# SerezD/vqvae-vqgan-pytorch-lightning

Hardware: AMD Instinct MI355X
Metric: images/sec/node (256x256 bs=32/GPU) VQ-VAE train step (higher is better)
Workload: dtype bf16; 1 GPU; standard_vqvae cb=1024, 256x256 bs=32/GPU (encoder+VQ+decoder fwd/bwd + AdamW); yaml=example_confs/standard_vqvae.yaml, global_batch=32, parallelism=dp1, launch=hipGraph replay (fwd+bwd) + eager all-reduce + AdamW, deterministic=False

## Files before the change

include/vqk.h:

```cpp
#ifndef VQK_H_
#define VQK_H_

#include <stddef.h>
#include <stdint.h>

#ifdef __cplusplus
extern "C" {
#endif

#define VQK_F32 0
#define VQK_BF16 1

enum vqk_status {
    VQK_OK = 0,
    VQK_ERR_SHAPE = -1,
    VQK_ERR_DTYPE = -2,
    VQK_ERR_ALIGN = -3,
    VQK_ERR_LAUNCH = -4,
    VQK_ERR_ARG = -5,
    VQK_ERR_WORKSPACE = -6
};

const char* vqk_status_str(int status);
int vqk_version(void);
// ... 162 lines not shown
int vqk_ctx_set_tile_queue(vqk_ctx* ctx, void* ws, int64_t ws_bytes);
int vqk_ctx_set_deterministic(vqk_ctx* ctx, int on, void* ws, int64_t ws_bytes);
int vqk_set_tuning(const char* name, int value);
int vqk_reset_tuning(void);
int vqk_tuning_count(void);
const char* vqk_tuning_name(int i);
int vqk_conv_set_block_caps(int stream_blocks, int wgrad_blocks);
int vqk_probe_stream_add(const float* src, float* dst, int64_t bytes, int blocks, int passes, int sleep, void* stream);
int vqk_calib_fill(void* w, int64_t bytes, void* stream);
int vqk_calib_mfma(const void* w, int64_t w_bytes, float* sink, int iters, int blocks, void* stream);
int64_t vqk_calib_mfma_flops(int iters, int blocks);
int vqk_calib_copy(const void* src, void* dst, int64_t bytes, void* stream);
int vqk_conv_pack_dgrad(const float* w, void* wt, int dtype, int cout, int cin, int ksize, void* stream);
int vqk_conv2d_wgrad(int dtype, const void* x, const void* dy, float* dw, int n, int h_in, int w_in, int cin,
                     int cout, int ksize, int ups, const void* zeros, void* stream);
int64_t vqk_conv2d_wgrad_edge_ws_bytes(void);
int vqk_conv2d_wgrad_edge(int dtype, const void* x, const void* dy, float* dw, void* ws, int64_t ws_bytes, int n, int h,
                          int w, int cin, int cout, const void* zeros, void* stream);
int vqk_conv2d_wgrad_edge_true(int dtype, const void* x, const void* dy, float* dw, void* ws, int64_t ws_bytes, int n, int h,
                               int w, int cin, int cout, int thin_true, const void* zeros, void* stream);
int vqk_conv2d_thin_out(int dtype, const void* x, const void* w, const float* bias, void* y, int n, int h, int wd, int cin,
                        int cout, int act, const void* zeros, void* stream);
int vqk_colsum(int dtype, const void* x, int64_t rows, int c, float* out, void* stream);
int vqk_colsum_lead(int dtype, const void* x, int64_t rows, int c, int c_out, float scale, float* out, void* stream);
int vqk_cast(const float* src, void* dst, int dtype, int64_t n, void* stream);

int vqk_gn_stats(int dtype, const void* x, int n, int64_t hw, int c, int groups, float eps,
                 double* acc, float* stats, void* stream);
int vqk_gn_apply(int dtype, const void* x, const float* stats, const float* w, const float* b, void* y,
                 int n, int64_t hw, int c, int groups, int silu, void* stream);
// ... 135 lines not shown
```

vqvae-vqgan-pytorch-lightning_amd/_native.py:

```python
from __future__ import annotations

import ctypes
import fcntl
import os
import subprocess
from ctypes import c_char_p, c_double, c_float, c_int, c_int32, c_int64, c_void_p, POINTER

_HERE = os.path.dirname(os.path.abspath(__file__))
_CSRC = os.path.join(_HERE, 'csrc')
_SO = os.environ.get('VQK_LIB') or os.path.join(_HERE, 'libvqk.so')
_lib = None

P = c_void_p
I, L, F = c_int, c_int64, c_float

_PROTOS = {
    'vqk_row_sqnorm_f32': [P, L, I, P, P],
    'vqk_vq_assign_f32': [P, P, P, P, L, I, I, I, P, P],
    'vqk_vq_assign_filtered_f32': [P, P, P, P, L, I, I, I, P, P, L, P],
    'vqk_probe_stream_add': [P, P, L, I, I, I, P],
    'vqk_calib_fill': [P, L, P],
    'vqk_calib_mfma': [P, L, P, I, I, P],
    'vqk_calib_copy': [P, P, L, P],
    'vqk_vq_prepare_f32': [P, I, I, P, L, P],
# ... 53 lines not shown
    'vqk_conv_set_variant': [I],
    'vqk_conv_set_block_caps': [I, I],
    'vqk_set_deterministic': [I, P, L],
    'vqk_set_scratch': [P, L],
    'vqk_set_tile_queue': [P, L],
    'vqk_ctx_create': [P],
    'vqk_ctx_destroy': [P],
    'vqk_ctx_make_current': [P],
    'vqk_ctx_set_scratch': [P, P, L],
    'vqk_ctx_set_tile_queue': [P, P, L],
    'vqk_ctx_set_deterministic': [P, I, P, L],
    'vqk_conv_pack_dgrad': [P, P, I, I, I, I, P],
    'vqk_conv2d_wgrad': [I, P, P, P, I, I, I, I, I, I, I, P, P],
    'vqk_conv2d_wgrad_pooled_dy': [I, P, P, P, I, I, I, I, I, F, P, P],
    'vqk_conv2d_wgrad_ups_phase': [I, P, P, P, I, I, I, I, I, F, P, P],
    'vqk_split_pair_f32': [P, P, L, I, P],
    'vqk_conv2d_fprop_x3_gnstats': [P, P, P, P, P, I, I, I, I, I, I, P, I, P, P],
    'vqk_conv2d_wgrad_x3': [P, P, P, I, I, I, I, I, I, F, P, P],
    'vqk_conv2d_wgrad_x3_f32': [P, P, P, I, I, I, I, I, I, F, P],
    'vqk_conv2d_wgrad_pooled_dy_phase': [I, P, P, P, I, I, I, I, I, F, P, P],
    'vqk_conv2d_wgrad_edge': [I, P, P, P, P, L, I, I, I, I, I, P, P],
    'vqk_conv2d_wgrad_edge_true': [I, P, P, P, P, L, I, I, I, I, I, I, P, P],
    'vqk_conv2d_thin_out': [I, P, P, P, P, I, I, I, I, I, I, P, P],
    'vqk_colsum': [I, P, L, I, P, P],
    'vqk_colsum_lead': [I, P, L, I, I, F, P, P],
    'vqk_cast': [P, P, I, L, P],
    'vqk_gn_stats': [I, P, I, L, I, I, F, P, P, P],
    'vqk_gn_apply': [I, P, P, P, P, P, I, L, I, I, I, P],
    'vqk_gn_forward': [I, P, P, P, P, P, P, I, L, I, I, F, I, P],
    'vqk_gn_forward_presummed': [I, P, P, P, P, P, P, I, L, I, I, F, I, P],
# ... 131 lines not shown
```

vqvae-vqgan-pytorch-lightning_amd/csrc/api.cpp:

```cpp
#include <stdint.h>
#include <new>
#include "common.h"

extern "C" {

const char* vqk_status_str(int status) {
    switch (status) {
        case VQK_OK: return "ok";
        case VQK_ERR_SHAPE: return "unsupported or inconsistent shape";
        case VQK_ERR_DTYPE: return "unsupported dtype";
        case VQK_ERR_ALIGN: return "pointer is not 16-byte aligned";
        case VQK_ERR_LAUNCH: return "kernel launch failed";
        case VQK_ERR_ARG: return "bad argument";
        case VQK_ERR_WORKSPACE: return "workspace too small";
        default: return "unknown status";
    }
}

int vqk_version(void) { return 1; }
const char* vqk_arch(void) { return "gfx950"; }

}

struct vqk_ctx {
// ... 83 lines not shown
    {"SK_MAXMB", 0, 0},
    {"UPS_PHASE", 0, 0},
    {"WGRAD_BLOCKS", 0, 0},
    {"WGMX", 0, 0},
    {"WGRAD_GEN_BLOCKS", 0, 0},
    {"WGRAD_NO_PW16", 0, 0},
    {"WGRAD_NO_P16K", 0, 0},
    {"MX_HALF", 0, 0},
    {"MX_HALF_HW", 0, 0},
    {"UPFIRDN_TILE", 0, 0},
    {"GN_BLOCKS_REDUCE", 0, 0},
    {"GN_BLOCKS_APPLY", 0, 0},
    {"GN_NT_MB", 0, 0},
    {"GN_NO_SMALL", 0, 0},
    {"WGMX_COEF_E4", 0, 0},
    {"GN_CLUSTER_MAX_HW", 0, 0},
    {"COMM_CUS", 0, 0},
    {"MX_QUARTER", 0, 0},
    {"MX_S2", 0, 0},
    {"MX_S2_DGRAD_MIN", 0, 0},
    {"VQ_LDS", 0, 0},
    {"UPS_MERGE", 0, 0},
    {"TILE_QUEUE", 0, 0},
    {"X3_WL", 0, 0},
    {"X3_WGRAD_COEF_E4", 0, 0},
    {"X3_WGRAD_FOLD", 0, 0},
    {"X3_WGRAD_PHASE", 0, 0},
    {"X3_WGRAD_PHASE_CAP_PCT", 0, 0},
    {"X3_WGRAD_PHASE_COEF_E4", 0, 0}
};
// ... 28 lines not shown
```

vqvae-vqgan-pytorch-lightning_amd/csrc/conv_geom.h:

```cpp
#pragma once
#include "common.h"

namespace vqkd {

struct ConvGeom {
    int n, h_in, w_in, h, w, cin, cout, ks, ups;
    int stride, pad, zs, vh, vw;
    float acc_scale, out_gain;
    int pool;
    float pool_scale;
    int m;
    int sub, sub_py, sub_px, sub_h, sub_w, nkh, nkw, khl[2], kwl[2];
    int wrow_chunks;
    int cpt;
    int kchunks;
    int tiles_m, tiles_n;
    double* gn_ws;
    int gn_cpg;
    int gn_part_nblk, gn_part_base;
    int ntap, tap_oy, tap_ox, src_s, src_a, src_b, dst_s, dst_a, dst_b;
    int tapw, dst_h, dst_w, s2;
    int phase_mode;
    int phase_rev;
    int dy_pool;
// ... 22 lines not shown
int& conv_force_variant();
int& conv_wgrad_blocks();

int launch_conv3x3_x3(const void* x, const void* w, const float* bias, const void* res, void* y, const void* zeros,
                      const ConvGeom& g, int act, int blocks_cap, hipStream_t st);
int launch_conv3x3_wgrad_x3(const void* x, const void* dy, float* dw, const ConvGeom& g, int blocks_cap, hipStream_t st);

int launch_conv3x3_thin_out_f32(const float* x, const float* w, const float* bias, const float* res, float* y, int n, int h, int wd,
                                int cin, int act, float acc_scale, float out_gain, hipStream_t st);
int launch_conv3x3_thin_in_f32(const float* x, const float* w, const float* bias, float* y, int n, int h, int wd, int cout, hipStream_t st);
int thin_wgrad_rows(int h, int w);
int launch_conv3x3_wgrad_thin_f32(int mode, const float* wide, const float* thin, float* dw, int n, int h, int w, int cw, float scale,
                                  hipStream_t st);

int launch_conv3x3_wgrad_mx(const void* x, const void* dy, float* dw, const void* zeros, const ConvGeom& g, int tiles,
                            int splits, int pps, hipStream_t st, float* part = nullptr);

}
```

vqvae-vqgan-pytorch-lightning_amd/csrc/conv_wgmx.hip:

```cpp
#include "conv_geom.h"

namespace {
using vqkd::ConvGeom;
using vqkd::xcd_remap;

#ifndef VQK_WGMX_NST
#define VQK_WGMX_NST 3
#endif
#ifndef VQK_WGMX_PIN
#define VQK_WGMX_PIN 1
#endif
#define SGB(mask, n) __builtin_amdgcn_sched_group_barrier(mask, n, 0)

__device__ __forceinline__ void glds16(const void* src, char* lds_wave_base) {
    __builtin_amdgcn_global_load_lds((const VQK_GLB void*)src, (VQK_LDS void*)lds_wave_base, 16, 0, 0);
}
__device__ __forceinline__ bf16x8_t tr_frag2(const char* p) {
    const s16x4 lo = __builtin_amdgcn_ds_read_tr16_b64_v4i16((VQK_LDS s16x4*)p);
    const s16x4 hi = __builtin_amdgcn_ds_read_tr16_b64_v4i16((VQK_LDS s16x4*)(p + 256));
    typedef __attribute__((ext_vector_type(8))) short s16x8;
    const s16x8 v = {lo[0], lo[1], lo[2], lo[3], hi[0], hi[1], hi[2], hi[3]};
    return __builtin_bit_cast(bf16x8_t, v);
}

// ... 227 lines not shown
    }
}

__global__ __launch_bounds__(256) void wgrad_mx_reduce_kernel(const float* __restrict__ part, float* __restrict__ dw, int tiles,
                                                              int splits, int cin) {
    const int tile = blockIdx.y, tiles_ci = cin >> 6;
    const int e = (int)(blockIdx.x * 256 + threadIdx.x);
    if (e >= 64 * 9 * 64) return;
    const int cil = e & 63, ct = e >> 6, col = ct / 9, t = ct - col * 9;
    const int tco = tile / tiles_ci, tci = tile - tco * tiles_ci;
    float s = 0.0f;
    for (int k = 0; k < splits; ++k) s += part[((int64_t)k * tiles + tile) * (64 * 9 * 64) + e];
    dw[((int64_t)(tco * 64 + col) * 9 + t) * cin + tci * 64 + cil] += s;
}

}

namespace vqkd {

int launch_conv3x3_wgrad_mx(const void* x, const void* dy, float* dw, const void* zeros, const ConvGeom& g, int tiles,
                            int splits, int pps, hipStream_t st, float* part) {
    if (g.fold && (g.dy_pool || part)) return VQK_ERR_ARG;
    if (g.dy_pool >= 2) {
        if (g.dy_pool > 7 || part || (g.dy_pool >= 6 && (splits & 3))) return VQK_ERR_ARG;
        static const hipError_t attr4 = hipFuncSetAttribute((const void*)conv3x3_wgrad_mx_kernel<4>,
                                                            hipFuncAttributeMaxDynamicSharedMemorySize, VQK_WGMX_NST * 40960);
        if (attr4 != hipSuccess) return VQK_ERR_LAUNCH;
        hipLaunchKernelGGL(conv3x3_wgrad_mx_kernel<4>, dim3((unsigned)tiles, (unsigned)splits), dim3(512), VQK_WGMX_NST * 40960, st,
                           (const bf16_raw*)x, (const bf16_raw*)dy, dw, (const char*)zeros, g, pps, part);
        return hipGetLastError() == hipSuccess ? VQK_OK : VQK_ERR_LAUNCH;
    }
    static const hipError_t attr = hipFuncSetAttribute((const void*)conv3x3_wgrad_mx_kernel<9>,
                                                       hipFuncAttributeMaxDynamicSharedMemorySize, VQK_WGMX_NST * 40960);
    (void)attr;
    hipLaunchKernelGGL(conv3x3_wgrad_mx_kernel<9>, dim3((unsigned)tiles, (unsigned)splits), dim3(512), VQK_WGMX_NST * 40960, st,
                       (const bf16_raw*)x, (const bf16_raw*)dy, dw, (const char*)zeros, g, pps, part);
    if (hipGetLastError() != hipSuccess) return VQK_ERR_LAUNCH;
    if (part) {
        hipLaunchKernelGGL(wgrad_mx_reduce_kernel, dim3((64 * 9 * 64) / 256, (unsigned)tiles), dim3(256), 0, st, (const float*)part, dw,
                           tiles, splits, g.cin);
        if (hipGetLastError() != hipSuccess) return VQK_ERR_LAUNCH;
    }
    return VQK_OK;
}

}
```

vqvae-vqgan-pytorch-lightning_amd/csrc/conv_wgrad.hip:

```cpp
#include "conv_geom.h"
#include <math.h>

namespace {

using vqkd::ConvGeom;
using vqkd::xcd_remap;

__device__ __forceinline__ void glds16(const void* src, char* lds_wave_base) {
    __builtin_amdgcn_global_load_lds((const VQK_GLB void*)src, (VQK_LDS void*)lds_wave_base, 16, 0, 0);
}

template <typename T> struct WgradFrag;

template <> struct WgradFrag<bf16_raw> {
    static constexpr int KP = 64;
    static constexpr int ROWB = 256;
    __device__ static __forceinline__ bf16x8_t frag(const char* tile, int k0, int cbase, int lane) {
        const int i = lane & 15, grp = (lane >> 4) & 1, kgrp = lane >> 5;
        const int col = cbase + 16 * grp + 4 * (i & 3);
        const int row = k0 + 8 * kgrp + (i >> 2);
        const int lc = col >> 3;
        const char* p0 = tile + row * ROWB + ((lc ^ ((row & 3) << 2)) << 4) + ((col & 7) << 1);
        const char* p1 = p0 + 4 * ROWB;
        const s16x4 lo = __builtin_amdgcn_ds_read_tr16_b64_v4i16((VQK_LDS s16x4*)p0);
// ... 554 lines not shown

__global__ __launch_bounds__(256) void wgrad_split_reduce_kernel(const float* __restrict__ part, int64_t elems, int splits,
                                                                 float* __restrict__ dw) {
    const int64_t i = (int64_t)blockIdx.x * 256 + threadIdx.x;
    if (i >= elems) return;
    float s = 0.f;
    for (int k = 0; k < splits; ++k) s += part[(int64_t)k * elems + i];
    dw[i] += s;
}

#define g_force_variant (vqkd::conv_force_variant())
#define g_wgrad_blocks (vqkd::conv_wgrad_blocks())
#define g_det (vqkd::det_state().on)
#define g_det_ws (vqkd::det_state().ws)
#define g_det_ws_bytes (vqkd::det_state().bytes)
inline int make_geom(ConvGeom& g, int dtype, int n, int h_in, int w_in, int cin, int cout, int ksize, int ups) {
    return vqkd::conv_make_geom(g, dtype, n, h_in, w_in, cin, cout, ksize, ups);
}

}

extern "C" {

static int wgrad_general(int dtype, const void* x, const void* dy, float* dw, int n, int h_in, int w_in, int cin, int cout,
                         int ksize, int stride, int pad, int mode, int h_out, int w_out, const void* zeros, void* stream,
                         int dy_pool = 0, float dy_scale = 1.0f, int fold = 0) {
    VQK_REQUIRE(x && dy && dw && zeros, VQK_ERR_ARG);
    VQK_REQUIRE(vqk_aligned16(x) && vqk_aligned16(dy) && vqk_aligned16(zeros), VQK_ERR_ALIGN);
    VQK_REQUIRE(mode >= 0 && mode <= 1 && (stride == 1 || stride == 2) && pad >= 0, VQK_ERR_ARG);
    ConvGeom g;
// ... 41 lines not shown
            const double coef = VQK_TUNE("WGMX_COEF_E4", 800) * 1e-4;
            const int comm = VQK_TUNE("COMM_CUS", 0);
            const int nph = dy_pool >= 6 ? 4 : 1;
            const int capm = (cap / 2 - comm) / nph > tiles ? (cap / 2 - comm) / nph : tiles;
            int sm = (int)(sqrt(coef * (double)g.m / tiles) + 0.5);
            if (sm > (capm + tiles - 1) / tiles) sm = (capm + tiles - 1) / tiles;
            if (sm > (total_patches + 3) / 4) sm = (total_patches + 3) / 4;
            float* part = nullptr;
            if (g_det) {
                const int64_t per_split = (int64_t)tiles * 64 * 9 * 64 * 4;
                const int fit = (int)(g_det_ws_bytes / per_split);
                if (sm > fit) sm = fit;
                part = sm >= 2 ? g_det_ws : nullptr;
            }
            if (sm < 1) sm = 1;
            const int ppm = (total_patches + sm - 1) / sm;
            sm = (total_patches + ppm - 1) / ppm;
            if (sm < 2) part = nullptr;
            ConvGeom gm = g;
            gm.dy_pool = dy_pool; gm.acc_scale = dy_scale; gm.fold = fold;
            return vqkd::launch_conv3x3_wgrad_mx(x, dy, dw, zeros, gm, tiles, sm * nph, ppm, vqk_stream(stream), part);
        }
        if (dy_pool || fold) return VQK_ERR_SHAPE;
        if (pw16 && (cin % 64) == 0 && (cout % 64) == 0 && !no_p16k) {
            static const hipError_t attr = hipFuncSetAttribute((const void*)conv3x3_wgrad_p16_kernel,
                                                               hipFuncAttributeMaxDynamicSharedMemorySize, 2 * 40960);
            (void)attr;
            hipLaunchKernelGGL(conv3x3_wgrad_p16_kernel, grid, dim3(256), 2 * 40960, vqk_stream(stream),
                               (const bf16_raw*)x, (const bf16_raw*)dy, dw, (const char*)zeros, g, pps);
        } else if (pw16) {
            static const hipError_t attr = hipFuncSetAttribute((const void*)conv3x3_wgrad_halo_kernel<true>,
                                                               hipFuncAttributeMaxDynamicSharedMemorySize, 2 * 40960);
            (void)attr;
            hipLaunchKernelGGL(conv3x3_wgrad_halo_kernel<true>, grid, dim3(256), 2 * 40960, vqk_stream(stream),
                               (const bf16_raw*)x, (const bf16_raw*)dy, dw, (const char*)zeros, g, pps);
        } else {
// ... 39 lines not shown
        hipLaunchKernelGGL(conv_wgrad_kernel<float>, grid, dim3(256), 32768, vqk_stream(stream), (const float*)x, (const float*)dy, dst, (const char*)zeros, g, pps, sstride);
    else if (db) {
        static const hipError_t attr = hipFuncSetAttribute((const void*)conv_wgrad_db_kernel, hipFuncAttributeMaxDynamicSharedMemorySize, 65536);
        if (attr != hipSuccess) return VQK_ERR_LAUNCH;
        hipLaunchKernelGGL(conv_wgrad_db_kernel, grid, dim3(256), 65536, vqk_stream(stream), (const bf16_raw*)x, (const bf16_raw*)dy, dst, (const char*)zeros, g, pps, sstride);
    } else {
        hipLaunchKernelGGL(conv_wgrad_kernel<bf16_raw>, grid, dim3(256), 32768, vqk_stream(stream), (const bf16_raw*)x, (const bf16_raw*)dy, dst, (const char*)zeros, g, pps, sstride);
    }
    if (det_split)
        hipLaunchKernelGGL(wgrad_split_reduce_kernel, dim3((unsigned)((dw_elems + 255) / 256)), dim3(256), 0, vqk_stream(stream),
                           (const float*)g_det_ws, dw_elems, splits, dw);
    VQK_CHECK_LAUNCH();
    return VQK_OK;
}

int vqk_conv2d_wgrad(int dtype, const void* x, const void* dy, float* dw, int n, int h_in, int w_in, int cin, int cout,
                     int ksize, int ups, const void* zeros, void* stream) {
    VQK_REQUIRE(ups == 0 || ups == 1, VQK_ERR_ARG);
    return wgrad_general(dtype, x, dy, dw, n, h_in, w_in, cin, cout, ksize, 1, ksize >> 1, ups, h_in << ups, w_in << ups,
                         zeros, stream);
}

int vqk_conv2d_wgrad_x3_f32(const float* x, const float* dy, float* dw, int n, int h_in, int w_in, int cin, int cout, int ups,
                            float scale, void* stream) {
    VQK_REQUIRE(x && dy && dw, VQK_ERR_ARG);
    VQK_REQUIRE(vqk_aligned16(x) && vqk_aligned16(dy), VQK_ERR_ALIGN);
    VQK_REQUIRE(ups == 0 || ups == 1 || ups == 2, VQK_ERR_ARG);
    VQK_REQUIRE(!g_det && g_force_variant != 0, VQK_ERR_SHAPE);
    ConvGeom g;
    if (ups == 2 || (ups == 1 && VQK_TUNE("X3_WGRAD_PHASE", 1) && (h_in % 8) == 0 && (w_in % 8) == 0)) {
// ... 68 lines not shown
```

vqvae-vqgan-pytorch-lightning_amd/ops.py:

```python
from __future__ import annotations

import os
import threading
import weakref

import numpy as _np
import torch

from . import _native

F32, BF16 = 0, 1
_CL = torch.channels_last


def dcode(dtype: torch.dtype) -> int:
    if dtype == torch.float32:
        return F32
    if dtype == torch.bfloat16:
        return BF16
    raise RuntimeError(f'vqk: unsupported dtype {dtype}')


def epc(dtype: torch.dtype) -> int:
    return 4 if dtype == torch.float32 else 8
# ... 747 lines not shown


def edge_wgrad_served(x, dy, ksize: int, ups: bool) -> bool:
    n, cin, h, w = x.shape
    return (_EDGE_WGRAD and x.dtype == torch.bfloat16 and ksize == 3 and not ups and (cin, dy.shape[1]) in ((8, 128), (128, 8))
            and (h * w) % 128 == 0 and (w % 128 == 0 or 128 % w == 0))


def raw_split_pair(t) -> torch.Tensor:
    n, c, h, w = t.shape
    out = empty_nhwc(n, 2 * c, h, w, torch.bfloat16, t.device)
    st = _timed('split_pair_kernel (HBM)', 0.0,
                lambda: _native.lib().vqk_split_pair_f32(t.data_ptr(), out.data_ptr(), n * h * w, c, _stream()), t.numel() * 8.0)
    _native.check(st, 'split_pair')
    return out


def raw_conv_wgrad(x, dy, ksize: int, ups: bool, out=None, thin_true: int = 8, x3: bool = False) -> torch.Tensor:
    n, cin, h, w = x.shape
    cout = dy.shape[1]
    dw = out if out is not None else \
        torch.zeros((cout, ksize, ksize, cin), dtype=torch.float32, device=x.device).permute(0, 3, 1, 2)
    flops = 2.0 * n * dy.shape[2] * dy.shape[3] * cout * cin * ksize * ksize
    if edge_wgrad_served(x, dy, ksize, ups):
        ws = _edge_ws(x.device)
        nbytes = (x.numel() + dy.numel()) * 2
        st = _timed('conv3x3_wgrad_thin_kernel<bf16>' + (f' {cin}->{cout}@{h}x{w}' if _EVENT_SHAPES else ''), 0.0,
                    lambda: _native.lib().vqk_conv2d_wgrad_edge_true(dcode(x.dtype), x.data_ptr(), dy.data_ptr(), dw.data_ptr(),
                                                                     ws.data_ptr(), ws.numel() * 4, n, h, w, cin, cout, int(thin_true),
                                                                     zero_page(x.device).data_ptr(), _stream()), nbytes)
# ... 21 lines not shown
            return dw
    if (ups and UPS_PHASE_WGRAD and _WGMX_ON and x.dtype == torch.bfloat16 and ksize == 3 and cin % 64 == 0 and cout % 64 == 0
            and w % 16 == 0 and h % 8 == 0 and not DETERMINISTIC):
        st = _timed('conv3x3_wgrad_mx_kernel<bf16>' + (f' {cin}->{cout}@{dy.shape[2]}x{dy.shape[3]} k{ksize} phase' if _EVENT_SHAPES else ''), flops,
                    lambda: _native.lib().vqk_conv2d_wgrad_ups_phase(dcode(x.dtype), x.data_ptr(), dy.data_ptr(), dw.data_ptr(), n, h, w,
                                                                     cin, cout, 1.0, zero_page(x.device).data_ptr(), _stream()),
                    launches=4, exec_flops=flops * 4.0 / 9.0)
        if st != _native.ERR_SHAPE:
            _native.check(st, 'conv2d_wgrad_ups_phase')
            return dw
    mxw = (_WGMX_ON and x.dtype == torch.bfloat16 and ksize == 3 and cin % 64 == 0 and cout % 64 == 0
           and dy.shape[3] % 16 == 0 and dy.shape[2] % 8 == 0)
    kname = 'conv3x3_wgrad_mx_kernel<bf16>' if mxw else f'conv_wgrad_kernel<{"f32" if x.dtype == torch.float32 else "bf16"}>'
    if _EVENT_SHAPES:
        kname += f' {cin}->{cout}@{dy.shape[2]}x{dy.shape[3]} k{ksize}'
    st = _timed(kname, flops,
                lambda: _native.lib().vqk_conv2d_wgrad(dcode(x.dtype), x.data_ptr(), dy.data_ptr(), dw.data_ptr(), n, h,
                                                       w, cin, cout, ksize, int(ups),
                                                       zero_page(x.device).data_ptr(), _stream()))
    _native.check(st, 'conv2d_wgrad')
    return dw


X3_WGRAD_PHASE = _native.switch('VQK_X3_WGRAD_PHASE', '1') != '0'


def raw_conv_wgrad_pooled_x3(x, dy_pooled, scale: float, out) -> bool:
    n, cin, h, w = x.shape
    cout = dy_pooled.shape[1]
    if (not X3_WGRAD_PHASE or x.dtype != torch.float32 or dy_pooled.dtype != torch.float32 or cin % 64 or cout % 64 or h % 16 or w % 16
            or DETERMINISTIC or tuple(dy_pooled.shape[2:]) != (h // 2, w // 2)):
        return False
    flops = 2.0 * n * h * w * cout * cin * 9
    st = _timed('conv3x3_wgrad_x3_kernel<f32 as 3 x bf16>' + (f' {cin}->{cout}@{h}x{w} k3 pooled-dy phase' if _EVENT_SHAPES else ''), flops,
# ... 8 lines not shown
def raw_conv_wgrad_pooled_dy(x, dy_pooled, scale: float, out) -> bool:
    n, cin, h, w = x.shape
    cout = dy_pooled.shape[1]
    if not (_WGMX_ON and x.dtype == torch.bfloat16 and cin % 64 == 0 and cout % 64 == 0 and w % 16 == 0 and h % 8 == 0):
        return False
    flops = 2.0 * n * h * w * cout * cin * 9
    if POOLED_WGRAD_PHASE and not DETERMINISTIC and (h // 2) % 8 == 0 and (w // 2) % 16 == 0:
        st = _timed('conv3x3_wgrad_mx_kernel<bf16>' + (f' {cin}->{cout}@{h}x{w} pooled-dy phase' if _EVENT_SHAPES else ''), flops,
                    lambda: _native.lib().vqk_conv2d_wgrad_pooled_dy_phase(dcode(x.dtype), x.data_ptr(), dy_pooled.data_ptr(), out.data_ptr(),
                                                                           n, h // 2, w // 2, cin, cout, float(scale),
                                                                           zero_page(x.device).data_ptr(), _stream()),
                    exec_flops=flops * 4.0 / 9.0)
        if st != _native.ERR_SHAPE:
            _native.check(st, 'conv2d_wgrad_pooled_dy_phase')
            return True
    st = _timed('conv3x3_wgrad_mx_kernel<bf16>' + (f' {cin}->{cout}@{h}x{w} pooled-dy' if _EVENT_SHAPES else ''), flops,
                lambda: _native.lib().vqk_conv2d_wgrad_pooled_dy(dcode(x.dtype), x.data_ptr(), dy_pooled.data_ptr(), out.data_ptr(),
                                                                 n, h, w, cin, cout, float(scale),
                                                                 zero_page(x.device).data_ptr(), _stream()))
    if st == _native.ERR_SHAPE:
        return False
    _native.check(st, 'conv2d_wgrad_pooled_dy')
    return True


def raw_colsum(x2d_rows: int, c: int, x, out=None, lead: int | None = None, scale: float = 1.0) -> torch.Tensor:
    out = out if out is not None else torch.zeros(c, dtype=torch.float32, device=x.device)
    _native.check(_native.lib().vqk_colsum_lead(dcode(x.dtype), x.data_ptr(), x2d_rows, c, c if lead is None else lead, float(scale),
                                                out.data_ptr(), _stream()), 'colsum')
    return out


def raw_cast(src_f32, dtype) -> torch.Tensor:
    if dtype == torch.float32:
# ... 965 lines not shown
```

vqvae-vqgan-pytorch-lightning_amd/trainer.py:

```python
from __future__ import annotations

import contextlib
import os
from typing import Iterable

import torch
import torch.distributed as dist

from . import _native, ops


GAN_OPT_OVERLAP = _native.switch('VQK_GAN_OPT_OVERLAP', '1') != '0'


def init_distributed(backend: str | None = None) -> tuple[int, int, int]:
    world = int(os.environ.get('WORLD_SIZE', '1'))
    rank = int(os.environ.get('RANK', '0'))
    local = int(os.environ.get('LOCAL_RANK', '0'))
    force = os.environ.get('VQK_FORCE_DIST') == '1'
    if (world > 1 or force) and not dist.is_initialized():
        os.environ.setdefault('MASTER_ADDR', '127.0.0.1')
        os.environ.setdefault('MASTER_PORT', '29500')
        if backend is None:
            backend = 'nccl' if torch.cuda.is_available() else 'gloo'
# ... 33 lines not shown
        return self.optimizers

    def train_batch(self, model, batch, batch_index: int):
        opt = self.optimizers[0]
        model.on_train_batch_start(batch, batch_index)
        if not getattr(model, 'automatic_optimization', True):
            loss = model.training_step(batch, batch_index)
            self.global_step += 1
            self._log_step(model)
            return loss
        opt.zero_grad()
        if self._use_split(model, opt):
            loss = self._split_step(model, opt, batch, batch_index)
        else:
            loss = model.training_step(batch, batch_index)
            loss.backward()
            self._finish_deferred(model, opt)
            opt.all_reduce_grads()
        self._log_grads(model, opt, 'autoencoder')
        opt.step()
        self.global_step += 1
        self._log_step(model)
        return loss

    @staticmethod
    def _slog(model):
        log = getattr(model, 'scalar_log', None)
        return None if (log is None or log.paused) else log

    def _slog_groups(self, model, log) -> None:
        opt = self.optimizers[0]
# ... 88 lines not shown
    def _ranges(opt, n_stages: int):
        total = opt.flat_g.numel()
        if n_stages == 3:
            return [(0, opt.front_numel), (opt.front_numel, opt.back_start), (opt.back_start, total)]
        return [(0, opt.front_numel), (opt.front_numel, total)]

    def _split_step(self, model, opt, batch, batch_index):
        model.split_backward = True
        try:
            loss = model.training_step(batch, batch_index)
        finally:
            model.split_backward = False
        stages = self._backward_halves(model)
        works = []
        for k, (stage, (lo, hi)) in enumerate(zip(stages, self._ranges(opt, len(stages)))):
            stage()
            if k == len(stages) - 1:
                self._finish_deferred(model, opt)
            if hi > lo:
                works.append(opt.all_reduce_range(lo, hi))
        for w in works:
            if w is not None:
                w.wait()
        return loss

    @staticmethod
    def _finish_deferred(model, opt):
        q = getattr(model, 'quantizer', None)
        if getattr(q, 'defer_update', False):
            q.finish_update(force_collective=opt.force_collective)

    def capture(self, model, example_batch, warmup: int = 3, preserve_state: bool = False):
        opt = self.optimizers[0]
        snap = self._snapshot(model) if preserve_state else None
        with self._image_logging_deferred(model) as logs, self._scalar_log_deferred(model):
            return self._capture(model, example_batch, warmup, snap, logs)

    @contextlib.contextmanager
    def _image_logging_deferred(self, model):
# ... 31 lines not shown
        if self._deferred_q is not None:
            self._deferred_q.defer_update = True
        self._graph = torch.cuda.CUDAGraph()
        self._graph2 = self._graph3 = None
        model.defer_usage_accumulation = True
        if logs:
            model.keep_recon_pair = True
        split = self._use_split(model, opt)
        try:
            if split:
                model.split_backward = True
                with torch.cuda.graph(self._graph, stream=side, capture_error_mode='thread_local'):
                    opt.zero_grad()
                    self._static_loss = model.training_step(self._static_in, 0)
                    stages = self._backward_halves(model)
                    stages[0]()
                self._graph2 = torch.cuda.CUDAGraph()
                with torch.cuda.graph(self._graph2, pool=self._graph.pool(), stream=side, capture_error_mode='thread_local'):
                    stages[1]()
                if len(stages) == 3:
                    self._graph3 = torch.cuda.CUDAGraph()
                    with torch.cuda.graph(self._graph3, pool=self._graph.pool(), stream=side, capture_error_mode='thread_local'):
                        stages[2]()
            else:
                with torch.cuda.graph(self._graph, stream=side, capture_error_mode='thread_local'):
                    opt.zero_grad()
                    self._static_loss = model.training_step(self._static_in, 0)
                    self._static_loss.backward()
        finally:
            model.defer_usage_accumulation = False
            model.split_backward = False
        self._static_hist = model.quantizer.last_hist
        self._static_pair = model._recon_pair if logs else None
        return self._graph

    def _capture_gan(self, model, example_batch, warmup: int, snap=None, logs: bool = False):
        ae_opt, disc_opt = self.optimizers
        self._static_in = example_batch.clone()
        self._gan_phase = self._gan_adversarial(model)
        side = self._cap_stream = torch.cuda.Stream()
        side.wait_stream(torch.cuda.current_stream())
        with torch.cuda.stream(side):
            ops._stream()
# ... 114 lines not shown
            if snap['rng'][0] is not None:
                torch.cuda.set_rng_state(snap['rng'][0])
            torch.set_rng_state(snap['rng'][1])
        if snap.get('logged') is not None:
            model.logged = snap['logged']
        if snap.get('scalar_log') is not None and getattr(model, 'scalar_log', None) is not None:
            model.scalar_log.restore(snap['scalar_log'])

    def _eager_step(self, model, batch, batch_index):
        opt = self.optimizers[0]
        opt.zero_grad()
        if self._use_split(model, opt):
            loss = self._split_step(model, opt, batch, batch_index)
        else:
            loss = model.training_step(batch, batch_index)
            loss.backward()
            self._finish_deferred(model, opt)
            opt.all_reduce_grads()
        opt.step()
        return loss

    def train_batch_graphed(self, model, batch, batch_index: int):
        if not getattr(model, 'automatic_optimization', True):
            return self._train_batch_gan_graphed(model, batch, batch_index)
        opt = self.optimizers[0]
        model.on_train_batch_start(batch, batch_index)
        if batch is not self._static_in:
            self._static_in.copy_(batch, non_blocking=True)
        ops.repack_owned(None)
        self._graph.replay()
        if self._graph2 is not None:
# ... 119 lines not shown
```

Measured before the change: 1176 images/sec.

## Defer split-K wgrad reductions into a shared slab and batch-reduce per backward stage

MX 3x3 weight-gradient convolutions now write their split-K partials into a per-optimizer slab instead of reducing right after each layer. A single multi-layer reduce kernel then sums every pending layer into the flat gradient buffer when each backward stage ends. A separate sqrt-based heuristic picks a larger split count for these deferred layers, exposing more parallelism across CUs. The cost is a large HBM slab (up to 2 GB by default), extra partial-sum write and read traffic, and slab growth that only happens on eager steps outside graph capture.

```diff
diff --git a/include/vqk.h b/include/vqk.h
--- a/include/vqk.h
+++ b/include/vqk.h
@@ -200,6 +200,9 @@
 int vqk_conv_pack_dgrad(const float* w, void* wt, int dtype, int cout, int cin, int ksize, void* stream);
 int vqk_conv2d_wgrad(int dtype, const void* x, const void* dy, float* dw, int n, int h_in, int w_in, int cin,
                      int cout, int ksize, int ups, const void* zeros, void* stream);
+int vqk_set_wgrad_slab(void* slab, int64_t slab_bytes);
+int vqk_wgrad_slab_taken(int* tiles, int* splits);
+int vqk_wgrad_slab_reduce(const int64_t* layers, int count, void* stream);
 int64_t vqk_conv2d_wgrad_edge_ws_bytes(void);
 int vqk_conv2d_wgrad_edge(int dtype, const void* x, const void* dy, float* dw, void* ws, int64_t ws_bytes, int n, int h,
                           int w, int cin, int cout, const void* zeros, void* stream);
diff --git a/vqvae-vqgan-pytorch-lightning_amd/_native.py b/vqvae-vqgan-pytorch-lightning_amd/_native.py
--- a/vqvae-vqgan-pytorch-lightning_amd/_native.py
+++ b/vqvae-vqgan-pytorch-lightning_amd/_native.py
@@ -91,6 +91,9 @@
     'vqk_conv2d_wgrad': [I, P, P, P, I, I, I, I, I, I, I, P, P],
     'vqk_conv2d_wgrad_pooled_dy': [I, P, P, P, I, I, I, I, I, F, P, P],
     'vqk_conv2d_wgrad_ups_phase': [I, P, P, P, I, I, I, I, I, F, P, P],
+    'vqk_set_wgrad_slab': [P, L],
+    'vqk_wgrad_slab_taken': [P, P],
+    'vqk_wgrad_slab_reduce': [P, I, P],
     'vqk_split_pair_f32': [P, P, L, I, P],
     'vqk_conv2d_fprop_x3_gnstats': [P, P, P, P, P, I, I, I, I, I, I, P, I, P, P],
     'vqk_conv2d_wgrad_x3': [P, P, P, I, I, I, I, I, I, F, P, P],
diff --git a/vqvae-vqgan-pytorch-lightning_amd/csrc/api.cpp b/vqvae-vqgan-pytorch-lightning_amd/csrc/api.cpp
--- a/vqvae-vqgan-pytorch-lightning_amd/csrc/api.cpp
+++ b/vqvae-vqgan-pytorch-lightning_amd/csrc/api.cpp
@@ -121,6 +121,8 @@
     {"GN_NT_MB", 0, 0},
     {"GN_NO_SMALL", 0, 0},
     {"WGMX_COEF_E4", 0, 0},
+    {"WGMX_SLAB_COEF_E4", 0, 0},
+    {"WGMX_SLAB_MAX_HW", 0, 0},
     {"GN_CLUSTER_MAX_HW", 0, 0},
     {"COMM_CUS", 0, 0},
     {"MX_QUARTER", 0, 0},
diff --git a/vqvae-vqgan-pytorch-lightning_amd/csrc/conv_geom.h b/vqvae-vqgan-pytorch-lightning_amd/csrc/conv_geom.h
--- a/vqvae-vqgan-pytorch-lightning_amd/csrc/conv_geom.h
+++ b/vqvae-vqgan-pytorch-lightning_amd/csrc/conv_geom.h
@@ -60,6 +60,10 @@
                                   hipStream_t st);
 
 int launch_conv3x3_wgrad_mx(const void* x, const void* dy, float* dw, const void* zeros, const ConvGeom& g, int tiles,
-                            int splits, int pps, hipStream_t st, float* part = nullptr);
+                            int splits, int pps, hipStream_t st, float* part = nullptr, bool reduce_now = true);
+
+struct SlabLayer { const float* slab; float* dw; int tiles, splits, cin, first_block; };
+constexpr int kSlabLayers = 64;
+int launch_wgrad_slab_reduce(const SlabLayer* layers, int count, hipStream_t st);
 
 }
diff --git a/vqvae-vqgan-pytorch-lightning_amd/csrc/conv_wgmx.hip b/vqvae-vqgan-pytorch-lightning_amd/csrc/conv_wgmx.hip
--- a/vqvae-vqgan-pytorch-lightning_amd/csrc/conv_wgmx.hip
+++ b/vqvae-vqgan-pytorch-lightning_amd/csrc/conv_wgmx.hip
@@ -265,12 +265,62 @@
     dw[((int64_t)(tco * 64 + col) * 9 + t) * cin + tci * 64 + cil] += s;
 }
 
+struct SlabTable { vqkd::SlabLayer l[vqkd::kSlabLayers]; int count; };
+typedef float f32x4_slab __attribute__((ext_vector_type(4)));
+
+__global__ __launch_bounds__(256) void wgrad_slab_reduce_kernel(const SlabTable tb) {
+    constexpr int TILE = 64 * 9 * 64, BPT = TILE / (256 * 4);
+    const int b = (int)blockIdx.x;
+    int li = 0;
+    for (int k = 1; k < tb.count; ++k) li = b >= tb.l[k].first_block ? k : li;
+    const float* __restrict__ slab = tb.l[li].slab;
+    float* __restrict__ dw = tb.l[li].dw;
+    const int tiles = tb.l[li].tiles, splits = tb.l[li].splits, cin = tb.l[li].cin;
+    const int lb = b - tb.l[li].first_block;
+    const int tile = lb / BPT;
+    const int e = ((lb - tile * BPT) * 256 + (int)threadIdx.x) * 4;
+    if (tile >= tiles) return;
+    const int tiles_ci = cin >> 6;
+    const int cil = e & 63, ct = e >> 6, col = ct / 9, t = ct - col * 9;
+    const int tco = tile / tiles_ci, tci = tile - tco * tiles_ci;
+    const int64_t stride = (int64_t)tiles * TILE;
+    const float* p = slab + (int64_t)tile * TILE + e;
+    f32x4_slab s = {0.0f, 0.0f, 0.0f, 0.0f};
+    int k = 0;
+    for (; k + 4 <= splits; k += 4) {
+        const f32x4_slab v0 = __builtin_nontemporal_load((const f32x4_slab*)(p + (int64_t)k * stride));
+        const f32x4_slab v1 = __builtin_nontemporal_load((const f32x4_slab*)(p + (int64_t)(k + 1) * stride));
+        const f32x4_slab v2 = __builtin_nontemporal_load((const f32x4_slab*)(p + (int64_t)(k + 2) * stride));
+        const f32x4_slab v3 = __builtin_nontemporal_load((const f32x4_slab*)(p + (int64_t)(k + 3) * stride));
+        s += v0; s += v1; s += v2; s += v3;
+    }
+    for (; k < splits; ++k) s += __builtin_nontemporal_load((const f32x4_slab*)(p + (int64_t)k * stride));
+    f32x4_slab* q = (f32x4_slab*)(dw + ((int64_t)(tco * 64 + col) * 9 + t) * cin + tci * 64 + cil);
+    *q = *q + s;
+}
+
 }
 
 namespace vqkd {
 
+int launch_wgrad_slab_reduce(const SlabLayer* layers, int count, hipStream_t st) {
+    if (count < 1 || count > kSlabLayers) return VQK_ERR_ARG;
+    SlabTable tb;
+    int blocks = 0;
+    for (int i = 0; i < kSlabLayers; ++i) {
+        tb.l[i] = i < count ? layers[i] : SlabLayer{nullptr, nullptr, 0, 0, 64, 0};
+        if (i < count) {
+            tb.l[i].first_block = blocks;
+            blocks += layers[i].tiles * 36;
+        }
+    }
+    tb.count = count;
+    hipLaunchKernelGGL(wgrad_slab_reduce_kernel, dim3((unsigned)blocks), dim3(256), 0, st, tb);
+    return hipGetLastError() == hipSuccess ? VQK_OK : VQK_ERR_LAUNCH;
+}
+
 int launch_conv3x3_wgrad_mx(const void* x, const void* dy, float* dw, const void* zeros, const ConvGeom& g, int tiles,
-                            int splits, int pps, hipStream_t st, float* part) {
+                            int splits, int pps, hipStream_t st, float* part, bool reduce_now) {
     if (g.fold && (g.dy_pool || part)) return VQK_ERR_ARG;
     if (g.dy_pool >= 2) {
         if (g.dy_pool > 7 || part || (g.dy_pool >= 6 && (splits & 3))) return VQK_ERR_ARG;
@@ -287,7 +337,7 @@
     hipLaunchKernelGGL(conv3x3_wgrad_mx_kernel<9>, dim3((unsigned)tiles, (unsigned)splits), dim3(512), VQK_WGMX_NST * 40960, st,
                        (const bf16_raw*)x, (const bf16_raw*)dy, dw, (const char*)zeros, g, pps, part);
     if (hipGetLastError() != hipSuccess) return VQK_ERR_LAUNCH;
-    if (part) {
+    if (part && reduce_now) {
         hipLaunchKernelGGL(wgrad_mx_reduce_kernel, dim3((64 * 9 * 64) / 256, (unsigned)tiles), dim3(256), 0, st, (const float*)part, dw,
                            tiles, splits, g.cin);
         if (hipGetLastError() != hipSuccess) return VQK_ERR_LAUNCH;
diff --git a/vqvae-vqgan-pytorch-lightning_amd/csrc/conv_wgrad.hip b/vqvae-vqgan-pytorch-lightning_amd/csrc/conv_wgrad.hip
--- a/vqvae-vqgan-pytorch-lightning_amd/csrc/conv_wgrad.hip
+++ b/vqvae-vqgan-pytorch-lightning_amd/csrc/conv_wgrad.hip
@@ -592,6 +592,12 @@
 #define g_det (vqkd::det_state().on)
 #define g_det_ws (vqkd::det_state().ws)
 #define g_det_ws_bytes (vqkd::det_state().bytes)
+struct SlabState { float* ws; int64_t bytes; int tiles, splits; };
+SlabState& slab_state() {
+    static thread_local SlabState s = {nullptr, 0, 0, 0};
+    return s;
+}
+#define g_slab (slab_state())
 inline int make_geom(ConvGeom& g, int dtype, int n, int h_in, int w_in, int cin, int cout, int ksize, int ups) {
     return vqkd::conv_make_geom(g, dtype, n, h_in, w_in, cin, cout, ksize, ups);
 }
@@ -663,12 +669,31 @@
                 part = sm >= 2 ? g_det_ws : nullptr;
             }
             if (sm < 1) sm = 1;
-            const int ppm = (total_patches + sm - 1) / sm;
+            int ppm = (total_patches + sm - 1) / sm;
             sm = (total_patches + ppm - 1) / ppm;
             if (sm < 2) part = nullptr;
+            SlabState& slab = g_slab;
+            slab.tiles = slab.splits = 0;
+            bool deferred = false;
+            const int slab_max_hw = VQK_TUNE("WGMX_SLAB_MAX_HW", 0);
+            if (slab.ws && !g_det && !fold && dy_pool <= 1 && vqk_aligned16(dw) && (slab_max_hw <= 0 || g.h * g.w <= slab_max_hw)) {
+                const double scoef = VQK_TUNE("WGMX_SLAB_COEF_E4", 4000) * 1e-4;
+                int ss = (int)(sqrt(scoef * (double)g.m / tiles) + 0.5);
+                if (ss > (capm + tiles - 1) / tiles) ss = (capm + tiles - 1) / tiles;
+                if (ss > (total_patches + 3) / 4) ss = (total_patches + 3) / 4;
+                if (ss < 1) ss = 1;
+                const int pps_s = (total_patches + ss - 1) / ss;
+                ss = (total_patches + pps_s - 1) / pps_s;
+                if (ss >= 2 && (int64_t)ss * tiles * 64 * 9 * 64 * 4 <= slab.bytes) {
+                    sm = ss; ppm = pps_s; part = slab.ws; deferred = true;
+                    slab.tiles = tiles; slab.splits = ss;
+                } else if (ss >= 2) {
+                    slab.tiles = tiles; slab.splits = -ss;
+                }
+            }
             ConvGeom gm = g;
             gm.dy_pool = dy_pool; gm.acc_scale = dy_scale; gm.fold = fold;
-            return vqkd::launch_conv3x3_wgrad_mx(x, dy, dw, zeros, gm, tiles, sm * nph, ppm, vqk_stream(stream), part);
+            return vqkd::launch_conv3x3_wgrad_mx(x, dy, dw, zeros, gm, tiles, sm * nph, ppm, vqk_stream(stream), part, !deferred);
         }
         if (dy_pool || fold) return VQK_ERR_SHAPE;
         if (pw16 && (cin % 64) == 0 && (cout % 64) == 0 && !no_p16k) {
@@ -738,6 +763,42 @@
     return VQK_OK;
 }
 
+int vqk_set_wgrad_slab(void* slab, int64_t slab_bytes) {
+    VQK_REQUIRE(!slab || slab_bytes >= 0, VQK_ERR_ARG);
+    VQK_REQUIRE(vqk_aligned16(slab), VQK_ERR_ALIGN);
+    g_slab = SlabState{slab ? (float*)slab : nullptr, slab ? slab_bytes : 0, 0, 0};
+    return VQK_OK;
+}
+
+int vqk_wgrad_slab_taken(int* tiles, int* splits) {
+    VQK_REQUIRE(tiles && splits, VQK_ERR_ARG);
+    *tiles = g_slab.tiles; *splits = g_slab.splits;
+    return VQK_OK;
+}
+
+int vqk_wgrad_slab_reduce(const int64_t* layers, int count, void* stream) {
+    VQK_REQUIRE(layers && count >= 0, VQK_ERR_ARG);
+    for (int i = 0; i < count; ++i) {
+        const int64_t* d = layers + 4 * i;
+        const int tiles = (int)(d[2] & 0xffffffff), splits = (int)(d[2] >> 32);
+        VQK_REQUIRE(d[0] && d[1] && tiles >= 1 && splits >= 1 && d[3] >= 64 && (d[3] % 64) == 0 && tiles % (int)(d[3] / 64) == 0
+                    && tiles <= (1 << 20), VQK_ERR_ARG);
+        VQK_REQUIRE(((uintptr_t)d[0] & 15) == 0 && ((uintptr_t)d[1] & 15) == 0, VQK_ERR_ALIGN);
+    }
+    for (int i0 = 0; i0 < count; i0 += vqkd::kSlabLayers) {
+        vqkd::SlabLayer tb[vqkd::kSlabLayers];
+        const int nl = count - i0 < vqkd::kSlabLayers ? count - i0 : vqkd::kSlabLayers;
+        for (int i = 0; i < nl; ++i) {
+            const int64_t* d = layers + 4 * (i0 + i);
+            tb[i] = vqkd::SlabLayer{(const float*)(uintptr_t)d[0], (float*)(uintptr_t)d[1], (int)(d[2] & 0xffffffff), (int)(d[2] >> 32),
+                                    (int)d[3], 0};
+        }
+        const int rc = vqkd::launch_wgrad_slab_reduce(tb, nl, vqk_stream(stream));
+        if (rc) return rc;
+    }
+    return VQK_OK;
+}
+
 int vqk_conv2d_wgrad(int dtype, const void* x, const void* dy, float* dw, int n, int h_in, int w_in, int cin, int cout,
                      int ksize, int ups, const void* zeros, void* stream) {
     VQK_REQUIRE(ups == 0 || ups == 1, VQK_ERR_ARG);
diff --git a/vqvae-vqgan-pytorch-lightning_amd/ops.py b/vqvae-vqgan-pytorch-lightning_amd/ops.py
--- a/vqvae-vqgan-pytorch-lightning_amd/ops.py
+++ b/vqvae-vqgan-pytorch-lightning_amd/ops.py
@@ -785,6 +785,134 @@
                 lambda: _native.lib().vqk_split_pair_f32(t.data_ptr(), out.data_ptr(), n * h * w, c, _stream()), t.numel() * 8.0)
     _native.check(st, 'split_pair')
     return out
+
+
+_WGRAD_SLAB_CAP = int(_native.switch('VQK_WGRAD_SLAB_MB', '2048')) << 20
+_WGRAD_DEFER_ON = _native.switch('VQK_WGRAD_DEFER', '1') != '0'
+_WGRAD_TILE_BYTES = 64 * 9 * 64 * 4
+_WGRAD_SESSIONS: list = []
+_WGRAD_LOCK = threading.Lock()
+
+
+class WgradDeferral:
+
+    def __init__(self, arena=None, cap_bytes: int | None = None):
+        self.range = None if arena is None else (arena.data_ptr(), arena.data_ptr() + arena.numel() * arena.element_size())
+        self.cap = _WGRAD_SLAB_CAP if cap_bytes is None else int(cap_bytes)
+        self.chunks: list = []
+        self.pending: dict = {}
+        self.unmet = 0
+        self.fallbacks = 0
+        self.flushed: list = []
+        self.depth = 0
+
+    def owns(self, out) -> bool:
+        return self.range is None or self.range[0] <= out.data_ptr() < self.range[1]
+
+    def slab_bytes(self) -> int:
+        return sum(c[0].numel() for c in self.chunks)
+
+    def reserve(self, nbytes: int, device=None) -> int:
+        nbytes = min(int(nbytes), self.cap - self.slab_bytes())
+        if nbytes >= 2 * _WGRAD_TILE_BYTES:
+            dev = torch.cuda.current_device() if device is None else device
+            with _WGRAD_LOCK:
+                self.chunks.append([torch.empty(nbytes, dtype=torch.uint8, device=dev), 0])
+        return self.slab_bytes()
+
+    def __enter__(self):
+        with _WGRAD_LOCK:
+            if self.depth == 0:
+                self.pending.clear()
+                for c in self.chunks:
+                    c[1] = 0
+                _WGRAD_SESSIONS.append(self)
+            self.depth += 1
+        return self
+
+    def __exit__(self, exc_type, exc, tb):
+        try:
+            if exc_type is None and self.depth == 1:
+                self.flush()
+        finally:
+            with _WGRAD_LOCK:
+                self.depth -= 1
+                if self.depth == 0:
+                    _WGRAD_SESSIONS.remove(self)
+                    self.pending.clear()
+        return False
+
+    def launch(self, out, cin: int, device, call):
+        import ctypes
+        lib = _native.lib()
+        with _WGRAD_LOCK:
+            key = out.data_ptr()
+            best = max(self.chunks, key=lambda c: c[0].numel() - c[1], default=None) if key not in self.pending else None
+        if key in self.pending:
+            self.fallbacks += 1
+            return call()
+        if best is None:
+            ptr, room = zero_page(device).data_ptr(), 0
+        else:
+            ptr, room = best[0].data_ptr() + best[1], best[0].numel() - best[1]
+        _native.check(lib.vqk_set_wgrad_slab(ptr, room), 'set_wgrad_slab')
+        try:
+            st = call()
+            tiles, splits = ctypes.c_int(0), ctypes.c_int(0)
+            _native.check(lib.vqk_wgrad_slab_taken(ctypes.byref(tiles), ctypes.byref(splits)), 'wgrad_slab_taken')
+        finally:
+            _native.check(lib.vqk_set_wgrad_slab(None, 0), 'set_wgrad_slab')
+        with _WGRAD_LOCK:
+            if st == 0 and tiles.value > 0 and splits.value > 0:
+                self.pending[key] = (ptr, tiles.value, splits.value, int(cin))
+                best[1] += (tiles.value * splits.value * _WGRAD_TILE_BYTES + 255) & ~255
+            else:
+                self.fallbacks += 1
+                if splits.value < 0:
+                    self.unmet += (tiles.value * -splits.value * _WGRAD_TILE_BYTES + 255) & ~255
+        return st
+
+    def flush(self) -> int:
+        import ctypes
+        with _WGRAD_LOCK:
+            layers = list(self.pending.items())
+            self.pending.clear()
+            for c in self.chunks:
+                c[1] = 0
+            unmet, self.unmet = self.unmet, 0
+        if layers:
+            words, nbytes = [], 0.0
+            for dw_ptr, (slab_ptr, tiles, splits, cin) in layers:
+                words += [slab_ptr, dw_ptr, tiles | (splits << 32), cin]
+                nbytes += float(tiles) * (splits + 2) * _WGRAD_TILE_BYTES
+            table = (ctypes.c_int64 * len(words))(*words)
+            st = _timed('wgrad_slab_reduce (HBM)', 0.0,
+                        lambda: _native.lib().vqk_wgrad_slab_reduce(table, len(layers), _stream()), nbytes)
+            _native.check(st, 'wgrad_slab_reduce')
+            self.flushed = [dw_ptr for dw_ptr, _ in layers]
+        if unmet and not torch.cuda.is_current_stream_capturing():
+            self.reserve(unmet)
+        return len(layers)
+
+
+def wgrad_deferral(arena=None, cap_bytes: int | None = None) -> WgradDeferral:
+    return WgradDeferral(arena, cap_bytes)
+
+
+def flush_wgrad() -> int:
+    with _WGRAD_LOCK:
+        open_now = list(_WGRAD_SESSIONS)
+    return sum(s.flush() for s in open_now)
+
+
+def _wgrad_session(out):
+    if out is None or not _WGRAD_SESSIONS or DETERMINISTIC:
+        return None
+    with _WGRAD_LOCK:
+        for s in _WGRAD_SESSIONS:
+            if s.owns(out):
+                return s
+    return None
 
 
 def raw_conv_wgrad(x, dy, ksize: int, ups: bool, out=None, thin_true: int = 8, x3: bool = False) -> torch.Tensor:
@@ -836,10 +964,11 @@
     kname = 'conv3x3_wgrad_mx_kernel<bf16>' if mxw else f'conv_wgrad_kernel<{"f32" if x.dtype == torch.float32 else "bf16"}>'
     if _EVENT_SHAPES:
         kname += f' {cin}->{cout}@{dy.shape[2]}x{dy.shape[3]} k{ksize}'
-    st = _timed(kname, flops,
-                lambda: _native.lib().vqk_conv2d_wgrad(dcode(x.dtype), x.data_ptr(), dy.data_ptr(), dw.data_ptr(), n, h,
-                                                       w, cin, cout, ksize, int(ups),
-                                                       zero_page(x.device).data_ptr(), _stream()))
+    def call():
+        return _native.lib().vqk_conv2d_wgrad(dcode(x.dtype), x.data_ptr(), dy.data_ptr(), dw.data_ptr(), n, h, w, cin, cout, ksize,
+                                              int(ups), zero_page(x.device).data_ptr(), _stream())
+    sess = _wgrad_session(out) if mxw else None
+    st = _timed(kname, flops, call if sess is None else (lambda: sess.launch(dw, cin, x.device, call)))
     _native.check(st, 'conv2d_wgrad')
     return dw
 
@@ -878,10 +1007,12 @@
         if st != _native.ERR_SHAPE:
             _native.check(st, 'conv2d_wgrad_pooled_dy_phase')
             return True
+    def call():
+        return _native.lib().vqk_conv2d_wgrad_pooled_dy(dcode(x.dtype), x.data_ptr(), dy_pooled.data_ptr(), out.data_ptr(), n, h, w, cin,
+                                                        cout, float(scale), zero_page(x.device).data_ptr(), _stream())
+    sess = _wgrad_session(out)
     st = _timed('conv3x3_wgrad_mx_kernel<bf16>' + (f' {cin}->{cout}@{h}x{w} pooled-dy' if _EVENT_SHAPES else ''), flops,
-                lambda: _native.lib().vqk_conv2d_wgrad_pooled_dy(dcode(x.dtype), x.data_ptr(), dy_pooled.data_ptr(), out.data_ptr(),
-                                                                 n, h, w, cin, cout, float(scale),
-                                                                 zero_page(x.device).data_ptr(), _stream()))
+                call if sess is None else (lambda: sess.launch(out, cin, x.device, call)))
     if st == _native.ERR_SHAPE:
         return False
     _native.check(st, 'conv2d_wgrad_pooled_dy')
diff --git a/vqvae-vqgan-pytorch-lightning_amd/trainer.py b/vqvae-vqgan-pytorch-lightning_amd/trainer.py
--- a/vqvae-vqgan-pytorch-lightning_amd/trainer.py
+++ b/vqvae-vqgan-pytorch-lightning_amd/trainer.py
@@ -71,7 +71,8 @@
             loss = self._split_step(model, opt, batch, batch_index)
         else:
             loss = model.training_step(batch, batch_index)
-            loss.backward()
+            with self._wgrad_deferred(model, opt):
+                loss.backward()
             self._finish_deferred(model, opt)
             opt.all_reduce_grads()
         self._log_grads(model, opt, 'autoencoder')
@@ -190,7 +191,8 @@
         stages = self._backward_halves(model)
         works = []
         for k, (stage, (lo, hi)) in enumerate(zip(stages, self._ranges(opt, len(stages)))):
-            stage()
+            with self._wgrad_deferred(model, opt):
+                stage()
             if k == len(stages) - 1:
                 self._finish_deferred(model, opt)
             if hi > lo:
@@ -199,6 +201,18 @@
             if w is not None:
                 w.wait()
         return loss
+
+    def _wgrad_deferred(self, model, opt):
+        if (not ops._WGRAD_DEFER_ON or ops.DETERMINISTIC or getattr(model, 'compute_dtype', None) != torch.bfloat16
+                or getattr(opt, 'flat_g', None) is None or not opt.flat_g.is_cuda):
+            return contextlib.nullcontext()
+        held = getattr(self, '_wgrad_sessions', None)
+        if held is None:
+            held = self._wgrad_sessions = {}
+        sess = held.get(id(opt))
+        if sess is None:
+            sess = held[id(opt)] = (opt, ops.wgrad_deferral(opt.flat_g))
+        return sess[1]
 
     @staticmethod
     def _finish_deferred(model, opt):
@@ -260,19 +274,23 @@
                     opt.zero_grad()
                     self._static_loss = model.training_step(self._static_in, 0)
                     stages = self._backward_halves(model)
-                    stages[0]()
+                    with self._wgrad_deferred(model, opt):
+                        stages[0]()
                 self._graph2 = torch.cuda.CUDAGraph()
                 with torch.cuda.graph(self._graph2, pool=self._graph.pool(), stream=side, capture_error_mode='thread_local'):
-                    stages[1]()
+                    with self._wgrad_deferred(model, opt):
+                        stages[1]()
                 if len(stages) == 3:
                     self._graph3 = torch.cuda.CUDAGraph()
                     with torch.cuda.graph(self._graph3, pool=self._graph.pool(), stream=side, capture_error_mode='thread_local'):
-                        stages[2]()
+                        with self._wgrad_deferred(model, opt):
+                            stages[2]()
             else:
                 with torch.cuda.graph(self._graph, stream=side, capture_error_mode='thread_local'):
                     opt.zero_grad()
                     self._static_loss = model.training_step(self._static_in, 0)
-                    self._static_loss.backward()
+                    with self._wgrad_deferred(model, opt):
+                        self._static_loss.backward()
         finally:
             model.defer_usage_accumulation = False
             model.split_backward = False
@@ -417,7 +435,8 @@
             loss = self._split_step(model, opt, batch, batch_index)
         else:
             loss = model.training_step(batch, batch_index)
-            loss.backward()
+            with self._wgrad_deferred(model, opt):
+                loss.backward()
             self._finish_deferred(model, opt)
             opt.all_reduce_grads()
         opt.step()
```

Result: no change. 1174 images/sec (-0.1%).
